# Iselix/kwiiyatta

Measured on AMD Instinct MI355X. Metric: frames/sec end-to-end analyse->align->convert->synth, 48 kHz 5 ms hop, higher is better.
Workload: dtype f64; 1 GPU; config3: 48 kHz source (10 s, T=2001) + target (11 s, T=2201) pairs: CheapTrick+D4C of both, pad with freshly drawn silent spectra, sp2mc, FastDTW(radius 32) align, GMM(64 comp, D=144)+MLPG convert, mc2sp, WORLD synthesis; pairs_per_gpu=32, streams_per_gpu=4, GPU_MAX_HW_QUEUES=4, launch=the whole step is one captured HIP graph, gmm_model_prepared=once per converter (the per-mixture matrices depend on the GMM only), parallelism=pairs in lockstep x32 per GPU, pair-per-GPU x1, no collective

## Files before the change

### kwiiyatta_amd/csrc/kwy_align.hip

```cpp
#include "kwy_internal.hpp"

__device__ __forceinline__ void align_features_body(const double *__restrict__ mc, int64_t T,
                                                    int ncoef, const double *__restrict__ f0,
                                                    double power_threshold, double power_weight,
                                                    double vuv_weight, double *__restrict__ out) {
  __shared__ double red[KWY_WAVES];
  const int tid = threadIdx.x;
  double mx = -INFINITY;
  for (int64_t t = tid; t < T; t += KWY_THREADS) mx = fmax(mx, mc[t * ncoef]);
#pragma unroll
  for (int o = 32; o > 0; o >>= 1) mx = fmax(mx, __shfl_down(mx, o));
  if ((tid & 63) == 0) red[tid >> 6] = mx;
  __syncthreads();
  double m = red[0];
  for (int i = 1; i < KWY_WAVES; ++i) m = fmax(m, red[i]);
  const double thr = m - power_threshold;
  const int64_t t = (int64_t)blockIdx.x * 8 + (tid >> 5);
  if (t >= T) return;
  const int w = ncoef + 1;
  for (int c = tid & 31; c < w; c += 32) {
    double v;
    if (c == 0) v = mc[t * ncoef] >= thr ? power_weight : 0.0;
    else if (c == 1) v = f0[t] > 0 ? vuv_weight : 0.0;
    else v = mc[t * ncoef + (c - 1)];
    out[t * w + c] = v;
  }
}

#define AL_TILE 1024
#define AL_NT 256
__device__ __forceinline__ void align_project_body(const int32_t *__restrict__ path,
                                                   const int64_t *__restrict__ path_len, int trim_len,
                                                   int32_t *__restrict__ idx, int64_t cap,
                                                   int64_t *__restrict__ n_out) {
  __shared__ int32_t sp[2 * AL_TILE];
  __shared__ int32_t so[AL_TILE];
  __shared__ long long st[5];
  __shared__ int s_irregular;
  const int tid = threadIdx.x, lane = tid & 63;
  const int64_t L = *path_len;
  if (L <= 0) { if (tid == 0) *n_out = 0; return; }
  long long len_y = path[2 * (L - 1) + 1] + 1;
  const long long prev_y0 = -1 + (trim_len > 0 ? trim_len : 0);
  if (trim_len > 0) len_y -= trim_len;
  if (tid == 0) s_irregular = 0;
  __syncthreads();
  {
    bool bad = false;
    for (int64_t k = tid; k < L; k += AL_NT) {
      const long long y = path[2 * k + 1], yp = k > 0 ? path[2 * k - 1] : -1;
      if (y < yp || y - yp > 1) bad = true;
    }
    if (bad) s_irregular = 1;
  }
  __syncthreads();
  if (!s_irregular) {
    for (int64_t k = tid; k < L; k += AL_NT) {
      const long long y = path[2 * k + 1], yp = k > 0 ? path[2 * k - 1] : -1;
      if (y > yp && y > prev_y0 && y < len_y) {
        const long long n = y - (prev_y0 + 1);
        if (n < cap) idx[n] = path[2 * k];
      }
    }
    if (tid == 0) { const long long n = len_y - (prev_y0 + 1); *n_out = n > 0 ? n : 0; }
    return;
  }
  if (tid >= 64) return;
  if (lane == 0) { st[0] = -1; st[1] = prev_y0; st[2] = 0; st[3] = 0; st[4] = 0; }
  int64_t k0 = 0;
  while (k0 < L) {
    const int nk = (int)min((int64_t)AL_TILE, L - k0);
    for (int e = lane; e < 2 * nk; e += 64) sp[e] = path[2 * k0 + e];
    __builtin_amdgcn_wave_barrier();
    __threadfence_block();
    __shared__ int s_used, s_made;
    if (lane == 0) {
      long long prev_x = st[0], prev_y = st[1];
      int made = 0, k = 0;
// ... 1 lines not shown
      for (; k < nk && !stop; ++k) {
        long long x = sp[2 * k], y = sp[2 * k + 1];
        if (y <= prev_y) continue;
        if (y - prev_y > 1) {
          if (y > len_y - 1) y = len_y - 1;
          const long long diff_x = x - prev_x, diff_y = y - prev_y;
          long long i = st[4];
          for (; i < diff_y && made < AL_TILE; ++i) {
            const long long den = diff_y - 1, num = diff_x * i;
            const long long q = den != 0 ? (num >= 0 ? num / den : -((-num + den - 1) / den)) : 0;
            so[made++] = (int32_t)(prev_x + q);
          }
          if (i < diff_y) { st[4] = i; break; }
          st[4] = 0;
        } else if (y >= len_y) {
          stop = true;
          break;
        } else {
          if (made >= AL_TILE) break;
          so[made++] = (int32_t)x;
        }
        prev_x = x;
        prev_y = y;
      }
      st[0] = prev_x; st[1] = prev_y;
      s_used = k; s_made = made;
      if (stop) st[3] = 1;
    }
    __builtin_amdgcn_wave_barrier();
    __threadfence_block();
    const int made = s_made, used = s_used;
    const long long n0 = st[2];
    for (int e = lane; e < made; e += 64)
      if (n0 + e < cap) idx[n0 + e] = so[e];
    __builtin_amdgcn_wave_barrier();
    if (lane == 0) st[2] = n0 + made;
    __builtin_amdgcn_wave_barrier();
    __threadfence_block();
    if (st[3]) break;
    if (used == 0 && made == 0) break;
    k0 += used;
  }
  if (lane == 0) *n_out = st[2];
}

#define AL_BATCH 64
template <class JOB>
struct al_jobs { int n; JOB j[AL_BATCH]; };

__global__ __launch_bounds__(KWY_THREADS) void k_align_features(al_jobs<kwy_align_job> b, int ncoef,
                                                               double power_threshold, double power_weight,
                                                               double vuv_weight) {
  const kwy_align_job &q = b.j[blockIdx.y];
  if ((int64_t)blockIdx.x * 8 >= q.T) return;
  align_features_body(q.mc, q.T, ncoef, q.f0, power_threshold, power_weight, vuv_weight, q.out);
}

__global__ __launch_bounds__(AL_NT) void k_align_project(al_jobs<kwy_project_job> b, int trim_len) {
  const kwy_project_job &q = b.j[blockIdx.x];
  align_project_body(q.path, q.path_len, trim_len, q.idx, q.idx_capacity, q.n_out);
}

__global__ void k_gather_rows(al_jobs<kwy_gather_job> b, int width) {
  const kwy_gather_job &q = b.j[blockIdx.y];
  const double *__restrict__ src = q.src;
  const int32_t *__restrict__ idx = q.idx;
  double *__restrict__ dst = q.dst;
  const int64_t src_rows = q.src_rows, n = q.n;
  const int64_t row = blockIdx.x;
  if (row >= n) return;
  int64_t r = idx[row];
  if (r < 0) r = 0;
  if (r >= src_rows) r = src_rows - 1;
  const double *s = src + r * width;
  double *d = dst + row * width;
  for (int c = threadIdx.x; c < width; c += blockDim.x) d[c] = s[c];
}

template <class JOB, class LAUNCH>
static int al_for_batches(const JOB *jobs, int count, LAUNCH launch) {
  for (int j0 = 0; j0 < count; j0 += AL_BATCH) {
    al_jobs<JOB> b;
    b.n = count - j0 < AL_BATCH ? count - j0 : AL_BATCH;
    for (int k = 0; k < AL_BATCH; ++k) b.j[k] = jobs[j0 + (k < b.n ? k : 0)];
    launch(b);
  }
  return KWY_OK;
}

extern "C" int kwy_align_features_batch_dev(kwy_ctx *ctx, const kwy_align_job *jobs, int count, int ncoef,
                                            double power_weight, double power_threshold, double vuv_weight) {
  if (!ctx) return KWY_EINVAL;
  if (!jobs || count < 0 || ncoef < 1) { ctx->err = "align_features: bad argument"; return KWY_EINVAL; }
  for (int j = 0; j < count; ++j)
    if (!jobs[j].mc || !jobs[j].f0 || !jobs[j].out || jobs[j].T <= 0) { ctx->err = "align_features: bad argument"; return KWY_EINVAL; }
  KWY_HIP(hipSetDevice(ctx->device));
  al_for_batches(jobs, count, [&](const al_jobs<kwy_align_job> &b) {
    int64_t T = 0;
    for (int k = 0; k < b.n; ++k) T = b.j[k].T > T ? b.j[k].T : T;
    hipLaunchKernelGGL(k_align_features, dim3((unsigned)((T + 7) / 8), b.n), dim3(KWY_THREADS), 0, ctx->stream, b, ncoef,
                       power_threshold, power_weight, vuv_weight);
  });
  KWY_HIP(hipGetLastError());
  return KWY_OK;
}

extern "C" int kwy_align_features_dev(kwy_ctx *ctx, const double *mc, int64_t T, int ncoef, const double *f0,
                                      double power_weight, double power_threshold, double vuv_weight,
                                      double *out) {
  const kwy_align_job job = {mc, f0, T, out};
  return kwy_align_features_batch_dev(ctx, &job, 1, ncoef, power_weight, power_threshold, vuv_weight);
}

extern "C" int kwy_align_project_batch_dev(kwy_ctx *ctx, const kwy_project_job *jobs, int count, int trim_len) {
  if (!ctx) return KWY_EINVAL;
  if (!jobs || count < 0 || trim_len < 0) { ctx->err = "align_project: bad argument"; return KWY_EINVAL; }
  for (int j = 0; j < count; ++j)
    if (!jobs[j].path || !jobs[j].path_len || !jobs[j].idx || !jobs[j].n_out || jobs[j].idx_capacity <= 0) {
      ctx->err = "align_project: bad argument";
      return KWY_EINVAL;
    }
  KWY_HIP(hipSetDevice(ctx->device));
  al_for_batches(jobs, count, [&](const al_jobs<kwy_project_job> &b) {
    hipLaunchKernelGGL(k_align_project, dim3(b.n), dim3(AL_NT), 0, ctx->stream, b, trim_len);
  });
  KWY_HIP(hipGetLastError());
  return KWY_OK;
}

extern "C" int kwy_align_project_dev(kwy_ctx *ctx, const int32_t *path, const int64_t *path_len, int trim_len,
                                     int32_t *idx, int64_t idx_capacity, int64_t *n_out) {
  const kwy_project_job job = {path, path_len, idx, idx_capacity, n_out};
  return kwy_align_project_batch_dev(ctx, &job, 1, trim_len);
}

extern "C" int kwy_gather_rows_batch_dev(kwy_ctx *ctx, const kwy_gather_job *jobs, int count, int width) {
  if (!ctx) return KWY_EINVAL;
  if (!jobs || count < 0 || width <= 0) { ctx->err = "gather_rows: bad argument"; return KWY_EINVAL; }
  for (int j = 0; j < count; ++j)
    if (!jobs[j].src || !jobs[j].idx || !jobs[j].dst || jobs[j].src_rows <= 0 || jobs[j].n < 0) {
      ctx->err = "gather_rows: bad argument";
      return KWY_EINVAL;
    }
  KWY_HIP(hipSetDevice(ctx->device));
  al_for_batches(jobs, count, [&](const al_jobs<kwy_gather_job> &b) {
    int64_t n = 0;
    for (int k = 0; k < b.n; ++k) n = b.j[k].n > n ? b.j[k].n : n;
    if (n > 0)
      hipLaunchKernelGGL(k_gather_rows, dim3((unsigned)n, b.n), dim3(width >= 256 ? 256 : 64), 0, ctx->stream, b, width);
  });
  KWY_HIP(hipGetLastError());
  return KWY_OK;
}
// ... 7 lines not shown
```

### kwiiyatta_amd/csrc/kwy_dtw.hip

```cpp
#include <math.h>

#include <algorithm>
#include <vector>

#include "kwy_internal.hpp"


__global__ void k_dtw_halve(const double *__restrict__ in, int n_out, int dim, double *__restrict__ out) {
  const int64_t e = (int64_t)blockIdx.x * blockDim.x + threadIdx.x;
  if (e >= (int64_t)n_out * dim) return;
  const int i = (int)(e / dim), k = (int)(e % dim);
  out[e] = (in[(int64_t)(2 * i) * dim + k] + in[(int64_t)(2 * i + 1) * dim + k]) / 2;
}

#define DTW_MAXLV 12

__device__ __forceinline__ int dtw_strip_steps16(const int32_t *lo, const int32_t *hi, int len_x, int k) {
  const int il = min(64 * k + 63, len_x - 1);
  return ((hi[il] - lo[64 * k] + 1 + 63) + 15) & ~15;
}
__device__ __forceinline__ uint64_t dtw_skew_index(uint64_t sbase, int s, int lane) {
  return sbase + ((uint64_t)(s >> 1) * 64 + (uint64_t)lane) * 2 + (uint64_t)(s & 1);
}
template <int NT>
// ... 7 lines not shown
  int32_t *firstj = (int32_t *)(tot + NT), *lastj = firstj + crows;
  if (table) {
    for (int p = threadIdx.x; p < cn; p += NT) {
      const int r = cpath[2 * p], j = cpath[2 * p + 1];
      if (p == 0 || cpath[2 * (p - 1)] != r) firstj[r] = j;
      if (p == cn - 1 || cpath[2 * (p + 1)] != r) lastj[r] = j;
    }
    __syncthreads();
  }
  for (int i = threadIdx.x; i < len_x; i += NT) {
    int l = 0, h = len_y - 1;
    if (table) {
      const int a = i / 2;
      const int fr = a - radius;
      const int jf = fr < crows ? firstj[max(fr, 0)] : lastj[crows - 1];
      const int jl = lastj[min(a + radius, crows - 1)];
      l = max(0, 2 * (jf - radius));
      h = min(len_y - 1, 2 * (jl + radius) + 1);
    } else if (cpath && cn > 0) {
      const int a = i / 2;
      int b0 = 0, b1 = cn;
      while (b0 < b1) { int mid = (b0 + b1) >> 1; if (cpath[2 * mid] >= a - radius) b1 = mid; else b0 = mid + 1; }
      const int first = min(b0, cn - 1);
      b0 = 0; b1 = cn;
      while (b0 < b1) { int mid = (b0 + b1) >> 1; if (cpath[2 * mid] > a + radius) b1 = mid; else b0 = mid + 1; }
      const int last = max(b0 - 1, 0);
      l = max(0, 2 * (cpath[2 * first + 1] - radius));
      h = min(len_y - 1, 2 * (cpath[2 * last + 1] + radius) + 1);
    }
    lo[i] = l;
    hi[i] = h;
  }
  __syncthreads();
  kwy_block_count_scan<NT>([&](int64_t i) -> uint64_t { return (uint64_t)(hi[i] - lo[i] + 1); }, len_x, off, tot);
  const int nstrips = (len_x + 63) / 64;
  kwy_block_count_scan<NT>([&](int64_t k) -> uint64_t { return 64ull * (uint64_t)dtw_strip_steps16(lo, hi, len_x, (int)k); },
                           nstrips, soff, tot);
  __syncthreads();
  if (threadIdx.x == 0 && (off[len_x] > cap_rows || soff[nstrips] > cap_skew)) atomicExch(status, 1);
}

#define DTW_WS_NT 1024
__device__ __forceinline__ void dtw_window_scan_first(int radius, int len_x, int len_y, int32_t *lo, int32_t *hi,
                                                      uint64_t *off, uint64_t *soff, uint64_t cap_rows,
                                                      uint64_t cap_skew, int *status, uint64_t *tot, size_t tot_bytes) {
  if (threadIdx.x < 16) status[threadIdx.x] = 0;
  __syncthreads();
  dtw_window_scan_body<DTW_WS_NT>((const int32_t *)nullptr, 0, radius, len_x, len_y, lo, hi, off, soff, cap_rows,
                                  cap_skew, status, (unsigned char *)tot, tot_bytes);
}

#define DTW_DT 32
#define DTW_DTP (DTW_DT + 1)
#define DTW_DIST_LDS (sizeof(double) * (64 + 80) * DTW_DTP)
__device__ __forceinline__ void dtw_dist_body(const double *x, const double *y, int dim, int len_x, int len_y,
                                              const int32_t *lo, const int32_t *hi, const uint64_t *soff,
                                              double *dist, const int *status, unsigned unit_first,
                                              unsigned unit_stride, unsigned char *lds) {
  double *xs = (double *)lds, *ys = xs + 64 * DTW_DTP;
  if (status[0] != 0) return;
  const int nstrips = (len_x + 63) / 64;
  const uint64_t total = soff[nstrips];
  const int lane = threadIdx.x & 63, sub = threadIdx.x >> 6;
  constexpr int PER = 16 / (KWY_THREADS / 64);
  for (uint64_t cell0 = (uint64_t)unit_first * 1024ull; cell0 < total; cell0 += (uint64_t)unit_stride * 1024ull) {
    int a = 0, b = nstrips - 1;
    while (a < b) { const int mid = (a + b + 1) >> 1; if (soff[mid] <= cell0) a = mid; else b = mid - 1; }
    const int k = a;
    const uint64_t sb = soff[k];
    const int s0 = (int)((cell0 - sb) >> 6);
    const int i = 64 * k + lane;
    const bool valid = i < len_x;
    const int jmin = lo[64 * k], l = valid ? lo[i] : 0, h = valid ? hi[i] : -1;
    const int jbase = jmin + s0 - 63;
    bool in[PER];
    double acc[PER];
    bool any = false;
#pragma unroll
    for (int q = 0; q < PER; ++q) {
      const int j = jmin + s0 + PER * sub + q - lane;
      in[q] = j >= l && j <= h;
      any = any || in[q];
      acc[q] = 0.0;
    }
    if (__syncthreads_or(any)) {
      for (int c0 = 0; c0 < dim; c0 += DTW_DT) {
        const int cw = min(DTW_DT, dim - c0);
        __syncthreads();
        for (int e = threadIdx.x; e < 64 * cw; e += KWY_THREADS) {
          const int r = e / cw, c = e - r * cw, ii = 64 * k + r;
          xs[r * DTW_DTP + c] = ii < len_x ? x[(int64_t)ii * dim + c0 + c] : 0.0;
        }
        for (int e = threadIdx.x; e < 79 * cw; e += KWY_THREADS) {
          const int r = e / cw, c = e - r * cw, jj = jbase + r;
          ys[r * DTW_DTP + c] = (jj >= 0 && jj < len_y) ? y[(int64_t)jj * dim + c0 + c] : 0.0;
        }
        __syncthreads();
#pragma unroll
        for (int q = 0; q < PER; ++q) {
          if (in[q]) {
            const double *xr = xs + lane * DTW_DTP, *yr = ys + (PER * sub + q + 63 - lane) * DTW_DTP;
            double t = acc[q];
            for (int c = 0; c < cw; ++c) { const double df = xr[c] - yr[c]; t += df * df; }
            acc[q] = t;
          }
        }
      }
    }
#pragma unroll
    for (int q = 0; q < PER; ++q)
      dist[dtw_skew_index(sb, s0 + PER * sub + q, lane)] = in[q] ? sqrt(acc[q]) : INFINITY;
    __syncthreads();
  }
}

__device__ __forceinline__ double dtw_wave_shr1(double v, double first) {
  const int lo = __builtin_amdgcn_update_dpp(__double2loint(first), __double2loint(v), 0x138, 0xf, 0xf, false);
  const int hi = __builtin_amdgcn_update_dpp(__double2hiint(first), __double2hiint(v), 0x138, 0xf, 0xf, false);
  return __hiloint2double(hi, lo);
}
__device__ __forceinline__ int dtw_wave_shr1_i32(int v, int first) {
  return __builtin_amdgcn_update_dpp(first, v, 0x138, 0xf, 0xf, false);
}
__device__ __forceinline__ double dtw_wave_rol1(double v) {
  const int lo = __builtin_amdgcn_mov_dpp(__double2loint(v), 0x134, 0xf, 0xf, false);
  const int hi = __builtin_amdgcn_mov_dpp(__double2hiint(v), 0x134, 0xf, 0xf, false);
  return __hiloint2double(hi, lo);
}

__device__ __forceinline__ double dtw_min_raw(double a, double b) {
  return fmin(a, b);
}

__device__ __forceinline__ uint64_t dtw_group_base(const uint64_t *__restrict__ off, int i) {
  return (off[i] >> 6) + (uint64_t)i;
}

struct dtw_level_args {
  int len_x, len_y;
  const int32_t *lo, *hi;
  const uint64_t *off;
  const uint64_t *soff;
  uint64_t cap_rows, cap_skew;
  double *dist;
  double *dval;
  uint64_t *predm;
  double *bnd_global;
  int32_t *path, *rev, *sinfo;
  int64_t *path_len;
  double *out_dist;
  int *status;
  long long *dbg;
  int lds_bytes;
  int next_len_x, next_len_y, radius;
  int32_t *lo_w, *hi_w;
  uint64_t *off_w, *soff_w;
  const double *x, *y;
  int dim;
};

#define DTW_OFFLV 32
struct dtw_pair {
  const double *x, *y;
  int Tx, Ty;
  double *dist;
// ... 7 lines not shown
  uint64_t stride;
  uint64_t cap_rows, cap_skew;
  uint64_t off_x[DTW_OFFLV], off_y[DTW_OFFLV];
  uint64_t off_dist, off_dval, off_soff, off_predm, off_lo, off_hi, off_off, off_bnd, off_pathA, off_pathB, off_rev,
      off_sinfo, off_lenA, off_lenB, off_status;
  int bnd_lds;
  long long *dbg;
  dtw_pair p[KWY_BATCH_MAX];
};
__host__ __device__ static inline int dtw_num_levels(int Tx, int Ty, int radius) {
  int n = 1;
  while (!(Tx < radius + 2 || Ty < radius + 2)) { Tx /= 2; Ty /= 2; ++n; }
  return n;
}
__device__ __forceinline__ bool dtw_make_args(const dtw_batch &b, int pi, int lev, bool with_series, dtw_level_args &a) {
  const dtw_pair &q = b.p[pi];
  const int nlev = dtw_num_levels(q.Tx, q.Ty, b.radius);
  if (lev >= nlev) return false;
  char *base = b.scratch + (uint64_t)pi * b.stride;
  a.len_x = q.Tx >> lev; a.len_y = q.Ty >> lev;
  a.lo = (int32_t *)(base + b.off_lo); a.hi = (int32_t *)(base + b.off_hi);
  a.off = (uint64_t *)(base + b.off_off); a.soff = (uint64_t *)(base + b.off_soff);
  a.cap_rows = b.cap_rows; a.cap_skew = b.cap_skew;
  a.dist = (double *)(base + b.off_dist); a.dval = (double *)(base + b.off_dval);
  a.predm = (uint64_t *)(base + b.off_predm);
  a.bnd_global = b.bnd_lds ? nullptr : (double *)(base + b.off_bnd);
  const bool top = lev == 0;
  a.path = top ? q.path : (int32_t *)(base + ((lev & 1) ? b.off_pathA : b.off_pathB));
  a.path_len = top ? q.path_len : (int64_t *)(base + ((lev & 1) ? b.off_lenA : b.off_lenB));
  a.rev = (int32_t *)(base + b.off_rev); a.sinfo = (int32_t *)(base + b.off_sinfo);
  a.out_dist = q.dist;
  a.status = (int *)(base + b.off_status);
  a.dbg = b.dbg;
  a.lds_bytes = b.lds_bytes;
  a.next_len_x = top ? 0 : q.Tx >> (lev - 1);
  a.next_len_y = top ? 0 : q.Ty >> (lev - 1);
  a.radius = b.radius;
  a.lo_w = (int32_t *)(base + b.off_lo); a.hi_w = (int32_t *)(base + b.off_hi);
  a.off_w = (uint64_t *)(base + b.off_off); a.soff_w = (uint64_t *)(base + b.off_soff);
  a.x = with_series ? (lev == 0 ? q.x : (const double *)(base + b.off_x[lev])) : nullptr;
  a.y = with_series ? (lev == 0 ? q.y : (const double *)(base + b.off_y[lev])) : nullptr;
  a.dim = b.dim;
  return true;
}

#define DTW_WAVES 4
#define DTW_CHUNK 16
#ifndef DTW_RING
#define DTW_RING 5
#endif
#ifndef DTW_BLK
#define DTW_BLK 16
#endif
typedef double dtw_d2 __attribute__((ext_vector_type(2), aligned(16)));

template <bool BND_LDS>
__device__ __forceinline__ void dtw_values_body(const dtw_level_args &a, unsigned char *bt ) {
  const long long t_start = a.dbg ? clock64() : 0;
  __shared__ long long s_prog[DTW_WAVES];
#define DTW_PROG_LOAD(b) __hip_atomic_load(&s_prog[b], __ATOMIC_RELAXED, __HIP_MEMORY_SCOPE_WORKGROUP)
#define DTW_PROG_STORE(b, v) __hip_atomic_store(&s_prog[b], (long long)(v), __ATOMIC_RELAXED, __HIP_MEMORY_SCOPE_WORKGROUP)
#define DTW_RELEASE() do { if (BND_LDS) __builtin_amdgcn_fence(__ATOMIC_RELEASE, "wavefront"); else __builtin_amdgcn_fence(__ATOMIC_RELEASE, "workgroup"); } while (0)
#define DTW_ACQUIRE() do { if (BND_LDS) __builtin_amdgcn_fence(__ATOMIC_ACQUIRE, "wavefront"); else __builtin_amdgcn_fence(__ATOMIC_ACQUIRE, "workgroup"); } while (0)
  const int lane = threadIdx.x & 63, wv = __builtin_amdgcn_readfirstlane(threadIdx.x >> 6);
  if (a.status[0] != 0) return;
  const int len_x = a.len_x, len_y = a.len_y;
  const int32_t *lo = a.lo, *hi = a.hi;
  const uint64_t *off = a.off;
  long long *dbg = a.dbg;
  const double INF = INFINITY;
  const int rowlen = len_y + 2;
  double *const lds_rows = (double *)bt;
  double *const bnd_global = a.bnd_global;
#define BROW(buf, ix) (BND_LDS ? lds_rows[(buf) * rowlen + (ix)] : bnd_global[(size_t)(buf) * rowlen + (ix)])
  if (threadIdx.x < DTW_WAVES) DTW_PROG_STORE(threadIdx.x, -1);
  if (dbg && lane == 0) dbg[16 + wv] = __builtin_amdgcn_s_getreg((31 << 11) | (0 << 6) | 4);
  __syncthreads();
  const int nstrips = (len_x + 63) / 64;
  for (int k = wv; k < nstrips; k += DTW_WAVES) {
    const int i0 = k * 64;
    const int i = i0 + lane;
    const bool valid = i < len_x;
    const int rl = valid ? lo[i] : 0, rh = valid ? hi[i] : -1;
    const int rw = rh - rl;
    const int ilast = min(i0 + 63, len_x - 1);
    const int L = ilast - i0;
    const int jmin = __builtin_amdgcn_readfirstlane(lo[i0]), jmax = __builtin_amdgcn_readfirstlane(hi[ilast]);
    const int plo = k > 0 ? __builtin_amdgcn_readfirstlane(lo[i0 - 1]) : 0;
    const int phi = k > 0 ? __builtin_amdgcn_readfirstlane(hi[i0 - 1]) : -1;
    const int pbuf = (k + DTW_WAVES - 1) % DTW_WAVES, nbuf = k % DTW_WAVES;
    const uint64_t sbv = a.soff[k];
    const uint64_t sb = ((uint64_t)(uint32_t)__builtin_amdgcn_readfirstlane((int)(sbv >> 32)) << 32) |
                        (uint64_t)(uint32_t)__builtin_amdgcn_readfirstlane((int)(uint32_t)sbv);
    const dtw_d2 *dbase = (const dtw_d2 *)(a.dist + sb) + lane;
    dtw_d2 *vbase = (dtw_d2 *)(a.dval + sb) + lane;
    double v1 = INF;
    double up_prev = INF;
    const int nsteps = (jmax - jmin + 1) + 63, nsteps16 = (nsteps + 15) & ~15;
    if (dbg && lane == 0 && k < 48) { dbg[64 + 4 * k] = clock64() - t_start; dbg[64 + 4 * k + 2] = nsteps; dbg[64 + 4 * k + 3] = jmin; }
    const int shift = lane + rl - jmin;
    const int shL = __builtin_amdgcn_readlane(shift, L), rwL = __builtin_amdgcn_readlane(rw, L);
    const int rhL = __builtin_amdgcn_readlane(rh, L);
    int sIn0 = (shL + DTW_BLK - 1) & ~(DTW_BLK - 1);
    const int sIn1 = (shL + rwL - (DTW_BLK - 1)) & ~(DTW_BLK - 1);
    if (sIn1 < sIn0) sIn0 = 0x40000000;
    const unsigned inSpan = sIn1 >= sIn0 ? (unsigned)(sIn1 - sIn0) : 0u;
    if (k == 0 && lane == 0 && jmin == 0) up_prev = 0.0;
// ... 463 lines not shown
  for (int s = sub; s < steps; s += DTW_WAVES) {
    const int j = jmin + s - lane;
    double d = INFINITY;
    if (j >= l && j <= h) {
      const double *yr = ys + j * dp;
      double acc = 0.0;
      for (int c = 0; c < dim; ++c) { const double df = xr[c] - yr[c]; acc += df * df; }
      d = sqrt(acc);
    }
    a.dist[dtw_skew_index(0, s, lane)] = d;
  }
}
__global__ __launch_bounds__(KWY_THREADS) void k_dtw_halve_all(dtw_batch b) {
  extern __shared__ double hb[];
  const dtw_pair &q = b.p[blockIdx.y];
  const int levels = dtw_num_levels(q.Tx, q.Ty, b.radius) - 1;
  if (levels < 1) return;
  const int C = 1 << levels, dim = b.dim;
  const int chunks0 = (q.Tx + C - 1) / C;
  if ((int)blockIdx.x >= chunks0 + (q.Ty + C - 1) / C) return;
  char *base = b.scratch + (uint64_t)blockIdx.y * b.stride;
  const int s = (int)blockIdx.x < chunks0 ? 0 : 1;
  const int c = s == 0 ? blockIdx.x : blockIdx.x - chunks0;
  const int n = s == 0 ? q.Tx : q.Ty;
  const double *src = s == 0 ? q.x : q.y;
  double *A = hb, *B = hb + (size_t)C * dim;
  const int64_t f0 = (int64_t)c * C;
  const int have = (int)min((int64_t)C, (int64_t)n - f0);
  for (int e = threadIdx.x; e < have * dim; e += KWY_THREADS) A[e] = src[f0 * dim + e];
  __syncthreads();
  for (int l = 1; l <= levels; ++l) {
    const int nl = n >> l, per = C >> l;
    const int i0 = c * per;
    const int cnt = min(per, nl - i0);
    double *out = (double *)(base + (s == 0 ? b.off_x[l] : b.off_y[l]));
    for (int e = threadIdx.x; e < cnt * dim; e += KWY_THREADS) {
      const int i = e / dim, k = e - i * dim;
      const double v = (A[(2 * i) * dim + k] + A[(2 * i + 1) * dim + k]) / 2;
      B[e] = v;
      out[(int64_t)(i0 + i) * dim + k] = v;
    }
    __syncthreads();
    double *t = A; A = B; B = t;
  }
}
__global__ __launch_bounds__(DTW_WS_NT) void k_dtw_window_scan(dtw_batch b, int lev) {
  __shared__ uint64_t tot[DTW_WS_NT];
  dtw_level_args a;
  const dtw_pair &q = b.p[blockIdx.x];
  if (lev != dtw_num_levels(q.Tx, q.Ty, b.radius) - 1 || !dtw_make_args(b, blockIdx.x, lev, false, a)) return;
  dtw_window_scan_first(b.radius, a.len_x, a.len_y, a.lo_w, a.hi_w, a.off_w, a.soff_w, a.cap_rows, a.cap_skew, a.status,
                        tot, sizeof(tot));
}
__global__ __launch_bounds__(KWY_THREADS) void k_dtw_dist(dtw_batch b, int lev) {
  __shared__ double tiles[(64 + 80) * DTW_DTP];
  dtw_level_args a;
  if (!dtw_make_args(b, blockIdx.y, lev, true, a)) return;
  dtw_dist_body(a.x, a.y, a.dim, a.len_x, a.len_y, a.lo, a.hi, a.soff, a.dist, a.status, blockIdx.x, gridDim.x,
                (unsigned char *)tiles);
}
template <bool BND_LDS>
__global__ __launch_bounds__(64 * DTW_WAVES) void k_dtw_values(dtw_batch b, int lev) {
  extern __shared__ unsigned char bt[];
  dtw_level_args a;
  if (!dtw_make_args(b, blockIdx.x, lev, false, a)) return;
  dtw_values_body<BND_LDS>(a, bt);
}
__global__ __launch_bounds__(DTW_CODES_THREADS) void k_dtw_codes(dtw_batch b, int lev) {
  extern __shared__ unsigned char bt[];
  dtw_level_args a;
  if (!dtw_make_args(b, blockIdx.y, lev, false, a)) return;
  if ((int)blockIdx.x >= (a.len_x + 63) / 64) return;
  dtw_codes_body<DTW_CODES_THREADS>(a, blockIdx.x, bt);
}
__global__ __launch_bounds__(DTW_TRACE_NT) void k_dtw_trace(dtw_batch b, int lev) {
  extern __shared__ unsigned char bt[];
  dtw_level_args a;
  if (!dtw_make_args(b, blockIdx.x, lev, false, a)) return;
  dtw_trace_body(a, bt);
}
__global__ __launch_bounds__(64 * DTW_WAVES) void k_dtw_small(dtw_batch b, int lev, int with_dist) {
  extern __shared__ unsigned char bt[];
  dtw_level_args a;
  if (!dtw_make_args(b, blockIdx.x, lev, with_dist != 0, a)) return;
  if (a.x) { dtw_dist_small(a, bt); __syncthreads(); }
  dtw_values_body<true>(a, bt);
  __syncthreads();
  const int nstrips = (a.len_x + 63) / 64;
  for (int k = 0; k < nstrips; ++k) dtw_codes_body<64 * DTW_WAVES>(a, k, bt);
  __syncthreads();
  dtw_trace_body(a, bt);
}

static uint64_t dtw_cap(int len_x, int len_y, int radius, bool full) {
  const uint64_t worst = (uint64_t)len_x * (uint64_t)len_y;
  if (full) return worst;
  const uint64_t r = (uint64_t)radius;
  const uint64_t bound = 2 * (2 * r + 1) * ((uint64_t)len_y + 2) + ((uint64_t)len_x + 2) * (4 * r + 2);
  return bound < worst ? bound : worst;
}
static uint64_t dtw_cap_skew(int len_x, int len_y, int radius, bool full) {
  const uint64_t strips = ((uint64_t)len_x + 63) / 64;
  const uint64_t worst = 64 * strips * ((uint64_t)len_y + 80);
  if (full) return worst;
  const uint64_t r = (uint64_t)radius, m = (31 + 2 * r) / 32 + 1;
  const uint64_t bound = 64 * (m * ((uint64_t)len_y + 2) + strips * (4 * r + 2 + 63 + 15 + 16));
  return bound < worst ? bound : worst;
}
// ... 44 lines not shown
  b.dbg = (long long *)ctx->dbg;
  for (int p = 0; p < n; ++p) status_out[p] = (int *)(b.scratch + (size_t)p * b.stride + b.off_status);
  int nlev[KWY_BATCH_MAX], top = 0;
  for (int p = 0; p < n; ++p) { nlev[p] = dtw_num_levels(pairs[p].Tx, pairs[p].Ty, radius); top = std::max(top, nlev[p]); }
  {
    const int levels = top - 1;
    const size_t halve_lds = levels > 0 ? sizeof(double) * (((size_t)3 << levels) / 2) * dim : 0;
    if (levels > 0 && levels <= DTW_MAXLV && halve_lds <= 64 * 1024) {
      unsigned chunks = 1;
      for (int p = 0; p < n; ++p) {
        const int C = 1 << (nlev[p] - 1);
        chunks = std::max(chunks, (unsigned)((pairs[p].Tx + C - 1) / C + (pairs[p].Ty + C - 1) / C));
      }
      hipLaunchKernelGGL(k_dtw_halve_all, dim3(chunks, n), dim3(KWY_THREADS), halve_lds, ctx->stream, b);
    } else {
      for (int p = 0; p < n; ++p) {
        const double *px = pairs[p].x, *py = pairs[p].y;
        char *base = b.scratch + (size_t)p * b.stride;
        for (int l = 1; l < nlev[p]; ++l) {
          const int lx = pairs[p].Tx >> l, ly = pairs[p].Ty >> l;
          double *cx = (double *)(base + b.off_x[l]), *cy = (double *)(base + b.off_y[l]);
          hipLaunchKernelGGL(k_dtw_halve, dim3((unsigned)(((size_t)lx * dim + 255) / 256)), dim3(256), 0, ctx->stream, px,
                             lx, dim, cx);
          hipLaunchKernelGGL(k_dtw_halve, dim3((unsigned)(((size_t)ly * dim + 255) / 256)), dim3(256), 0, ctx->stream, py,
                             ly, dim, cy);
          px = cx; py = cy;
        }
      }
    }
  }
  const size_t bnd_bytes = sizeof(double) * DTW_WAVES * (Ty + 2);
  b.bnd_lds = bnd_bytes <= 150 * 1024 ? 1 : 0;
  const size_t big_lds = 150 * 1024;
  KWY_HIP(hipFuncSetAttribute((const void *)k_dtw_values<true>, hipFuncAttributeMaxDynamicSharedMemorySize, (int)big_lds));
  KWY_HIP(hipFuncSetAttribute((const void *)k_dtw_codes, hipFuncAttributeMaxDynamicSharedMemorySize, (int)big_lds));
  KWY_HIP(hipFuncSetAttribute((const void *)k_dtw_trace, hipFuncAttributeMaxDynamicSharedMemorySize, (int)big_lds));
  KWY_HIP(hipFuncSetAttribute((const void *)k_dtw_small, hipFuncAttributeMaxDynamicSharedMemorySize, (int)big_lds));

  for (int l = top - 1; l >= 0; --l) {
    int len_x = 0, len_y = 0;
    bool first = false, small = b.bnd_lds != 0, small_dist = true;
    for (int p = 0; p < n; ++p) {
      if (l >= nlev[p]) continue;
      const int lx = pairs[p].Tx >> l, ly = pairs[p].Ty >> l;
      len_x = std::max(len_x, lx); len_y = std::max(len_y, ly);
      first = first || l == nlev[p] - 1;
      small = small && (lx + 63) / 64 <= DTW_SMALL_STRIPS;
      small_dist = small_dist && sizeof(double) * (size_t)(lx + ly) * (size_t)(dim | 1) <= 96 * 1024;
    }
    small_dist = small_dist && small;
    if (first)
      hipLaunchKernelGGL(k_dtw_window_scan, dim3(n), dim3(DTW_WS_NT), 0, ctx->stream, b, l);
    const int nstrips = (len_x + 63) / 64;
    const uint64_t lv_units = std::min(b.cap_skew, dtw_cap_skew(len_x, len_y, radius, full)) / 1024 + 1;
    b.lds_bytes = 0;
    if (!small_dist)
      KWY_PROF(ctx, "k_dtw_dist", hipLaunchKernelGGL(k_dtw_dist, dim3((unsigned)lv_units, n), dim3(KWY_THREADS), 0, ctx->stream, b, l));
    if (small) {
      const size_t dist_b = small_dist ? sizeof(double) * (size_t)(len_x + len_y) * (size_t)(dim | 1) : 0;
      const size_t bnd_b = sizeof(double) * DTW_WAVES * ((size_t)len_y + 2);
      const size_t groups = 64 * ((size_t)len_y / 64 + 2);
      const size_t codes_b = (size_t)64 * 4 * (size_t)std::min<int64_t>(len_y, 8 * (int64_t)radius + 128) + 32 * groups;
      const size_t trace_b = 16 * ((size_t)len_x + 2) + 8 * DTW_TRACE_NT + 16 * groups + 256;
      size_t need = std::max(std::max(dist_b, bnd_b), std::max(codes_b, trace_b)) + 4096;
      need = std::min(big_lds, (need + 1023) & ~(size_t)1023);
      b.lds_bytes = (int)need;
      KWY_PROF(ctx, "k_dtw_small", hipLaunchKernelGGL(k_dtw_small, dim3(n), dim3(64 * DTW_WAVES), need, ctx->stream, b, l,
                                                       small_dist ? 1 : 0));
      continue;
    }
    const size_t want = (size_t)64 * 4 * (size_t)std::min<int64_t>(len_y, 8 * (int64_t)radius + 128);
    const size_t codes_lds = std::min(big_lds, std::max<size_t>(want, 16 * 1024));
    if (b.bnd_lds)
      KWY_PROF(ctx, "k_dtw_values", hipLaunchKernelGGL(k_dtw_values<true>, dim3(n), dim3(64 * DTW_WAVES), bnd_bytes, ctx->stream, b, l));
    else
      KWY_PROF(ctx, "k_dtw_values", hipLaunchKernelGGL(k_dtw_values<false>, dim3(n), dim3(64 * DTW_WAVES), 0, ctx->stream, b, l));
    b.lds_bytes = (int)codes_lds;
    KWY_PROF(ctx, "k_dtw_codes", hipLaunchKernelGGL(k_dtw_codes, dim3(nstrips, n), dim3(DTW_CODES_THREADS), codes_lds, ctx->stream, b, l));
    b.lds_bytes = (int)big_lds;
    KWY_PROF(ctx, "k_dtw_trace", hipLaunchKernelGGL(k_dtw_trace, dim3(n), dim3(DTW_TRACE_NT), big_lds, ctx->stream, b, l));
  }
  KWY_HIP(hipGetLastError());
  return KWY_OK;
}

static int dtw_check(kwy_ctx *ctx, const void *x, int64_t Tx, const void *y, int64_t Ty, int dim, int radius,
                     const void *dist, const void *path, const void *path_len) {
  if (!ctx) return KWY_EINVAL;
  if (!x || !y || !dist || !path || !path_len || Tx <= 0 || Ty <= 0 || dim <= 0 || dim > 4096 || radius < 0 ||
      Tx > 0x3fffffff || Ty > 0x3fffffff) {
    ctx->err = "fastdtw: bad argument";
    return KWY_EINVAL;
  }
  if (radius < 1) { ctx->err = "fastdtw: radius must be >= 1"; return KWY_EINVAL; }
  return KWY_OK;
}

extern "C" int kwy_fastdtw_batch_dev(kwy_ctx *ctx, const kwy_dtw_job *jobs, int count, int dim, int radius) {
  if (!ctx) return KWY_EINVAL;
  if (!jobs || count < 0) { ctx->err = "fastdtw_batch: bad argument"; return KWY_EINVAL; }
  if (count == 0) return KWY_OK;
  int64_t Tx = 0, Ty = 0;
  for (int j = 0; j < count; ++j) {
    KWY_TRY(dtw_check(ctx, jobs[j].x, jobs[j].x_length, jobs[j].y, jobs[j].y_length, dim, radius, jobs[j].dist,
                      jobs[j].path, jobs[j].path_len));
    Tx = std::max(Tx, jobs[j].x_length); Ty = std::max(Ty, jobs[j].y_length);
  }
// ... 60 lines not shown
```

### kwiiyatta_amd/csrc/kwy_synth.hip

```cpp
#include <math.h>
#include <stdlib.h>

#include <algorithm>
#include <vector>

#include "kwy_internal.hpp"

#define SYN_SAFE 0.000000000001
#define SYN_DEFAULT_F0 500.0
#define SYN_TILE_PER_THREAD 4
#define SYN_TILE (KWY_THREADS * SYN_TILE_PER_THREAD)
#define SYN_TWO_PI (2.0 * KWY_PI)
#define SYN_SLOTS(y_length, fs) ((int)((y_length) * 640 / (fs)) + 64)

struct syn_params {
  int64_t T, y_length;
  int fs, fft_size;
  double frame_period;
  double lowest_f0;
  double sp_mul;
};

__device__ __forceinline__ double syn_increment(const double *__restrict__ f0, const syn_params &p,
                                                int64_t n, double *vuv_out) {
// ... 996 lines not shown
          const double im2 = sqrt(1.0 - re2 * re2);
          buf[k] = {__builtin_fma(re, re2, im * im2), __builtin_fma(im, re2, -(re * im2))};
        }
      } else {
#pragma unroll
        for (int r = 0; r < RK; ++r) {
          const int k = tid + NT * r;
          if (k <= H) buf[k] = cmulf(mp[r], buf[k]);
        }
      }
      SYN_STAMP(3 + 5 * part);
      syn_irfft_inplace<LOG2N - 1, NT, V>(buf, twl, twP, twb, twN);
      SYN_STAMP(4 + 5 * part);
      if (part == 0) {
        const double *w = (const double *)buf;
        double ps[V];
#pragma unroll
        for (int g = 0; g < V; ++g) {
          ps[g] = 0.0;
          for (int i = tid + NT * g; i < H; i += KWY_THREADS) ps[g] += w[i];
        }
        dc_component = syn_block_sum_v<NT, V>(ps, red);
        SYN_STAMP(5);
      }
    }
    {
      const int tid = kwy_tid_opaque();
      SYN_STAMP(10);
      const double *w = (const double *)buf;
      const double sqrt_noise_size = sqrt((double)noise_size);
      double *slot = DIRECT ? nullptr : resp + (size_t)(pp - first_pulse) * N;
      const int64_t offset = (int64_t)idx - H + 1;
#pragma unroll
      for (int m = 0; m < C; ++m) {
        int i = tid + NT * m;
        double aper = (i < H) ? w[i + H] : w[i - H];
        double pv = 0.0;
        if (has_periodic) pv = (i < H) ? -dc_component * dc_remover[i] : lap[i - H] - dc_component * dc_remover[i];
        const double r = (pv * sqrt_noise_size + aper) / N;
        if constexpr (DIRECT) {
          const int64_t n = offset + i;
          if (n >= 0 && n < p.y_length) y[n] += r;
        } else {
          slot[i] = r;
        }
      }
      SYN_STAMP(11);
    }
  }
#undef SYN_STAMP
}


__global__ __launch_bounds__(KWY_THREADS) void k_syn_ola(syn_batch batch, int N) {
  const int utt = batch.find(blockIdx.x);
  const double *__restrict__ resp = batch.u[utt].resp;
  const int32_t *__restrict__ pidx = batch.u[utt].pidx;
  const int *__restrict__ tile_off = batch.u[utt].tile_off;
  const int *__restrict__ npulse = batch.u[utt].npulse;
  const int cap = batch.u[utt].cap, nt = batch.u[utt].nt, first_pulse = 0, slots = batch.u[utt].slots;
  const int64_t y_length = batch.u[utt].p.y_length;
  double *__restrict__ y = batch.u[utt].y;
  const int H = N / 2;
  const int tile = (int)blockIdx.x - batch.start[utt];
  const int P = min(npulse[0], cap);
  if (first_pulse >= P && first_pulse > 0) return;
  const int reach = (H + SYN_TILE - 1) / SYN_TILE;
  const int ja = max(0, tile - reach), jb = min(nt - 1, tile + reach);
  int p0 = min(tile_off[ja], P), p1 = jb + 1 < nt ? min(tile_off[jb + 1], P) : P;
  p0 = max(p0, first_pulse);
  p1 = min(p1, first_pulse + slots);
  const int64_t n0 = (int64_t)tile * SYN_TILE + threadIdx.x;
  double v[SYN_TILE_PER_THREAD];
#pragma unroll
  for (int m = 0; m < SYN_TILE_PER_THREAD; ++m) {
    const int64_t n = n0 + KWY_THREADS * m;
    v[m] = (first_pulse > 0 && n < y_length) ? y[n] : 0.0;
  }
  for (int pp = p0; pp < p1; ++pp) {
    const int idx = pidx[pp];
    if (pidx[min(P - 1, pp + 1)] - idx <= 0) continue;
    const double *slot = resp + (size_t)(pp - first_pulse) * N;
    const int64_t base = (int64_t)idx - H + 1;
#pragma unroll
    for (int m = 0; m < SYN_TILE_PER_THREAD; ++m) {
      const int64_t q = n0 + KWY_THREADS * m - base;
      if (q >= 0 && q < N) v[m] += slot[q];
    }
  }
#pragma unroll
  for (int m = 0; m < SYN_TILE_PER_THREAD; ++m) {
    const int64_t n = n0 + KWY_THREADS * m;
    if (n < y_length) y[n] = v[m];
  }
}

static int get_dc_remover(kwy_ctx *ctx, int fft_size, const double **out) {
  std::string key = "dcrem:" + std::to_string(fft_size);
  return kwy_cached_table<double>(ctx, key, [&] {
    std::vector<double> h(fft_size);
    double dc_component = 0.0;
    for (int i = 0; i < fft_size / 2; ++i) {
      h[i] = 0.5 - 0.5 * cos(2.0 * KWY_PI * (i + 1.0) / (1.0 + fft_size));
      h[fft_size - i - 1] = h[i];
      dc_component += h[i] * 2.0;
    }
    for (int i = 0; i < fft_size / 2; ++i) {
      h[i] /= dc_component;
      h[fft_size - i - 1] = h[i];
    }
    return h;
  }, out);
}

template <int LOG2N>
static int launch_pulse(kwy_ctx *ctx, syn_batch &batch) {
  constexpr int N = 1 << LOG2N, H = N / 2, K = H + 1;
  const kwy_c *twH, *twN, *twP;
  const uint4 *poly;
  const double *dcrem;
  KWY_TRY(kwy_get_twiddles(ctx, LOG2N - 1, &twH));
  KWY_TRY(kwy_get_twiddle_powers(ctx, LOG2N - 1, &twP));
  KWY_TRY(kwy_get_twiddles(ctx, LOG2N, &twN));
  KWY_TRY(kwy_get_poly(ctx, 12ull * (N / syn_pulse_nt<LOG2N>::value), &poly));
  KWY_TRY(get_dc_remover(ctx, N, &dcrem));
  constexpr int NT = syn_pulse_nt<LOG2N>::value;
  static_assert(K + 1 == syn_pulse_form<LOG2N>::H + 2, "the log-spectrum rows");
  size_t lds = syn_pulse_form<LOG2N>::lds;
  KWY_HIP(hipFuncSetAttribute((const void *)k_syn_pulse<LOG2N, false>,
                              hipFuncAttributeMaxDynamicSharedMemorySize, (int)lds));
  KWY_HIP(hipFuncSetAttribute((const void *)k_syn_pulse<LOG2N, true>,
                              hipFuncAttributeMaxDynamicSharedMemorySize, (int)lds));
  const int share = batch.n > 1 ? std::max(64, 4096 / batch.n) : 2048;
  int g = 0;
  for (int u = 0; u < batch.n; ++u) { batch.start[u] = g; g += std::max(1, std::min(batch.u[u].slots, share)); }
  batch.start[batch.n] = g;
  KWY_PROF(ctx, "k_syn_pulse", hipLaunchKernelGGL((k_syn_pulse<LOG2N, false>), dim3(g), dim3(NT), lds, ctx->stream, batch,
                     kwy_randn(ctx), poly, twH, twP, twN, dcrem, (long long *)ctx->dbg));
  g = 0;
  for (int u = 0; u < batch.n; ++u) { batch.start[u] = g; g += batch.u[u].nt; }
// ... 301 lines not shown
```

Measured before the change: 2.858 million frames/s.

## Retile DTW distance kernel, batch OLA pulse loads, widen align feature blocks

The DTW distance kernel now gives each work unit a variable run of anti-diagonal steps. It keeps the x rows in registers, accumulates pairs of cells with 2-wide vector stores across column chunks, and finds the strip with a block-parallel search. The synth overlap-add stages pulse indices in shared memory and issues loads for several pulses before accumulating, which raises memory-level parallelism. Align feature extraction now has each block handle 64 frames with a flat, coalesced write loop. These changes cut redundant LDS reloads and serial dependent loads, at the cost of more register pressure and extra read-modify-write passes over the distance buffer for each column chunk.

```diff
diff --git a/kwiiyatta_amd/csrc/kwy_align.hip b/kwiiyatta_amd/csrc/kwy_align.hip
--- a/kwiiyatta_amd/csrc/kwy_align.hip
+++ b/kwiiyatta_amd/csrc/kwy_align.hip
@@ -1,5 +1,8 @@
 #include "kwy_internal.hpp"
 
+#ifndef AL_FEAT_FRAMES
+#define AL_FEAT_FRAMES 64
+#endif
 __device__ __forceinline__ void align_features_body(const double *__restrict__ mc, int64_t T,
                                                     int ncoef, const double *__restrict__ f0,
                                                     double power_threshold, double power_weight,
@@ -7,6 +10,7 @@
   __shared__ double red[KWY_WAVES];
   const int tid = threadIdx.x;
   double mx = -INFINITY;
+#pragma unroll 8
   for (int64_t t = tid; t < T; t += KWY_THREADS) mx = fmax(mx, mc[t * ncoef]);
 #pragma unroll
   for (int o = 32; o > 0; o >>= 1) mx = fmax(mx, __shfl_down(mx, o));
@@ -15,15 +19,23 @@
   double m = red[0];
   for (int i = 1; i < KWY_WAVES; ++i) m = fmax(m, red[i]);
   const double thr = m - power_threshold;
-  const int64_t t = (int64_t)blockIdx.x * 8 + (tid >> 5);
-  if (t >= T) return;
   const int w = ncoef + 1;
-  for (int c = tid & 31; c < w; c += 32) {
+  const int64_t t0 = (int64_t)blockIdx.x * AL_FEAT_FRAMES;
+  const int64_t t1 = t0 + AL_FEAT_FRAMES < T ? t0 + AL_FEAT_FRAMES : T;
+  const int n = (int)(t1 - t0) * w;
+  const int dq = KWY_THREADS / w, dr = KWY_THREADS % w;
+  int tl = tid / w, c = tid % w;
+  double *__restrict__ dst = out + t0 * w;
+#pragma unroll 4
+  for (int e = tid; e < n; e += KWY_THREADS) {
+    const int64_t t = t0 + tl;
     double v;
     if (c == 0) v = mc[t * ncoef] >= thr ? power_weight : 0.0;
     else if (c == 1) v = f0[t] > 0 ? vuv_weight : 0.0;
     else v = mc[t * ncoef + (c - 1)];
-    out[t * w + c] = v;
+    dst[e] = v;
+    tl += dq; c += dr;
+    if (c >= w) { c -= w; ++tl; }
   }
 }
 
@@ -131,7 +143,7 @@
                                                                double power_threshold, double power_weight,
                                                                double vuv_weight) {
   const kwy_align_job &q = b.j[blockIdx.y];
-  if ((int64_t)blockIdx.x * 8 >= q.T) return;
+  if ((int64_t)blockIdx.x * AL_FEAT_FRAMES >= q.T) return;
   align_features_body(q.mc, q.T, ncoef, q.f0, power_threshold, power_weight, vuv_weight, q.out);
 }
 
@@ -177,7 +189,8 @@
   al_for_batches(jobs, count, [&](const al_jobs<kwy_align_job> &b) {
     int64_t T = 0;
     for (int k = 0; k < b.n; ++k) T = b.j[k].T > T ? b.j[k].T : T;
-    hipLaunchKernelGGL(k_align_features, dim3((unsigned)((T + 7) / 8), b.n), dim3(KWY_THREADS), 0, ctx->stream, b, ncoef,
+    hipLaunchKernelGGL(k_align_features, dim3((unsigned)((T + AL_FEAT_FRAMES - 1) / AL_FEAT_FRAMES), b.n), dim3(KWY_THREADS), 0,
+                       ctx->stream, b, ncoef,
                        power_threshold, power_weight, vuv_weight);
   });
   KWY_HIP(hipGetLastError());
diff --git a/kwiiyatta_amd/csrc/kwy_dtw.hip b/kwiiyatta_amd/csrc/kwy_dtw.hip
--- a/kwiiyatta_amd/csrc/kwy_dtw.hip
+++ b/kwiiyatta_amd/csrc/kwy_dtw.hip
@@ -83,65 +83,115 @@
 
 #define DTW_DT 32
 #define DTW_DTP (DTW_DT + 1)
-#define DTW_DIST_LDS (sizeof(double) * (64 + 80) * DTW_DTP)
+#ifndef DTW_RUN
+#define DTW_RUN 64
+#endif
+#define DTW_YROWS (DTW_RUN + 63)
+#define DTW_DIST_ROWS (DTW_YROWS + 1)
+#define DTW_DIST_LDS (sizeof(double) * DTW_DIST_ROWS * DTW_DTP)
+typedef double dtw_d2 __attribute__((ext_vector_type(2), aligned(16)));
+__host__ __device__ static inline uint64_t dtw_dist_units(uint64_t cells, uint64_t strips) {
+  return cells / (64ull * DTW_RUN) + strips + 1;
+}
+template <int CW>
+__device__ __forceinline__ void dtw_dist_pair(const double (&xr)[DTW_DT], const double *yr, double &a0, double &a1) {
+#pragma unroll
+  for (int c = 0; c < CW; ++c) {
+    if (c % 8 == 0) __builtin_amdgcn_sched_barrier(0);
+    const double d0 = xr[c] - yr[c], d1 = xr[c] - yr[DTW_DTP + c];
+    a0 += d0 * d0;
+    a1 += d1 * d1;
+  }
+}
 __device__ __forceinline__ void dtw_dist_body(const double *x, const double *y, int dim, int len_x, int len_y,
                                               const int32_t *lo, const int32_t *hi, const uint64_t *soff,
                                               double *dist, const int *status, unsigned unit_first,
                                               unsigned unit_stride, unsigned char *lds) {
-  double *xs = (double *)lds, *ys = xs + 64 * DTW_DTP;
-  if (status[0] != 0) return;
+  static_assert(DTW_RUN % 16 == 0 && DTW_RUN / 2 % KWY_WAVES == 0 && DTW_DIST_ROWS >= 64, "the run's thread map");
+  static_assert(KWY_THREADS % DTW_DT == 0 && DTW_DIST_ROWS % (8 * (KWY_THREADS / DTW_DT)) == 0, "the staging map");
+  double *tile = (double *)lds;
   const int nstrips = (len_x + 63) / 64;
-  const uint64_t total = soff[nstrips];
+  const int overflow = status[0];
+  const uint64_t nunits = soff[nstrips] / (64ull * DTW_RUN) + (uint64_t)nstrips;
+  if (overflow != 0) return;
   const int lane = threadIdx.x & 63, sub = threadIdx.x >> 6;
-  constexpr int PER = 16 / (KWY_THREADS / 64);
-  for (uint64_t cell0 = (uint64_t)unit_first * 1024ull; cell0 < total; cell0 += (uint64_t)unit_stride * 1024ull) {
+  const int scol = threadIdx.x & (DTW_DT - 1), srow = threadIdx.x / DTW_DT;
+  constexpr int SROWS = KWY_THREADS / DTW_DT;
+  constexpr int XP = 64 / SROWS, YP = DTW_DIST_ROWS / SROWS;
+  for (uint64_t u = unit_first; u < nunits; u += unit_stride) {
     int a = 0, b = nstrips - 1;
-    while (a < b) { const int mid = (a + b + 1) >> 1; if (soff[mid] <= cell0) a = mid; else b = mid - 1; }
-    const int k = a;
-    const uint64_t sb = soff[k];
-    const int s0 = (int)((cell0 - sb) >> 6);
+    while (b - a >= KWY_THREADS) {
+      const int mid = (a + b + 1) >> 1;
+      if (soff[mid] / (64ull * DTW_RUN) + (uint64_t)mid <= u) a = mid; else b = mid - 1;
+    }
+    const int cand = a + (int)threadIdx.x;
+    const int k = a - 1 + __syncthreads_count(cand <= b && soff[cand] / (64ull * DTW_RUN) + (uint64_t)cand <= u);
+    const uint64_t sb = soff[k], sb_next = soff[k + 1];
     const int i = 64 * k + lane;
     const bool valid = i < len_x;
     const int jmin = lo[64 * k], l = valid ? lo[i] : 0, h = valid ? hi[i] : -1;
+    const int steps16 = (int)((sb_next - sb) >> 6);
+    const int s0 = (int)(u - (sb / (64ull * DTW_RUN) + (uint64_t)k)) * DTW_RUN;
+    if (s0 >= steps16) continue;
+    const int nst = min(DTW_RUN, steps16 - s0);
     const int jbase = jmin + s0 - 63;
-    bool in[PER];
-    double acc[PER];
-    bool any = false;
-#pragma unroll
-    for (int q = 0; q < PER; ++q) {
-      const int j = jmin + s0 + PER * sub + q - lane;
-      in[q] = j >= l && j <= h;
-      any = any || in[q];
-      acc[q] = 0.0;
-    }
-    if (__syncthreads_or(any)) {
-      for (int c0 = 0; c0 < dim; c0 += DTW_DT) {
-        const int cw = min(DTW_DT, dim - c0);
-        __syncthreads();
-        for (int e = threadIdx.x; e < 64 * cw; e += KWY_THREADS) {
-          const int r = e / cw, c = e - r * cw, ii = 64 * k + r;
-          xs[r * DTW_DTP + c] = ii < len_x ? x[(int64_t)ii * dim + c0 + c] : 0.0;
+    dtw_d2 *band = (dtw_d2 *)(dist + sb) + lane;
+    for (int c0 = 0; c0 < dim; c0 += DTW_DT) {
+      const int cw = min(DTW_DT, dim - c0), cwp = (cw + 3) & ~3;
+      const bool first = c0 == 0, last = c0 + DTW_DT >= dim;
+      double xv[XP];
+#pragma unroll
+      for (int q = 0; q < XP; ++q) {
+        const int ii = 64 * k + srow + SROWS * q;
+        xv[q] = (scol < cw && ii < len_x) ? x[(int64_t)ii * dim + c0 + scol] : 0.0;
+      }
+      __syncthreads();
+      if (scol < cwp) {
+#pragma unroll
+        for (int q = 0; q < XP; ++q) tile[(srow + SROWS * q) * DTW_DTP + scol] = xv[q];
+      }
+      __syncthreads();
+      double xr[DTW_DT];
+#pragma unroll
+      for (int c = 0; c < DTW_DT; ++c) xr[c] = tile[lane * DTW_DTP + c];
+      __syncthreads();
+      if (scol < cwp) {
+#pragma unroll
+        for (int q0 = 0; q0 < YP; q0 += 8) {
+          double yv[8];
+#pragma unroll
+          for (int q = 0; q < 8; ++q) {
+            const int r = srow + SROWS * (q0 + q), jj = jbase + r;
+            yv[q] = (scol < cw && r < nst + 63 && jj >= 0 && jj < len_y) ? y[(int64_t)jj * dim + c0 + scol] : 0.0;
+          }
+#pragma unroll
+          for (int q = 0; q < 8; ++q) tile[(srow + SROWS * (q0 + q)) * DTW_DTP + scol] = yv[q];
         }
-        for (int e = threadIdx.x; e < 79 * cw; e += KWY_THREADS) {
-          const int r = e / cw, c = e - r * cw, jj = jbase + r;
-          ys[r * DTW_DTP + c] = (jj >= 0 && jj < len_y) ? y[(int64_t)jj * dim + c0 + c] : 0.0;
-        }
-        __syncthreads();
-#pragma unroll
-        for (int q = 0; q < PER; ++q) {
-          if (in[q]) {
-            const double *xr = xs + lane * DTW_DTP, *yr = ys + (PER * sub + q + 63 - lane) * DTW_DTP;
-            double t = acc[q];
-            for (int c = 0; c < cw; ++c) { const double df = xr[c] - yr[c]; t += df * df; }
-            acc[q] = t;
+      }
+      __syncthreads();
+      for (int p = sub; 2 * p < nst; p += KWY_WAVES) {
+        const int j0 = jmin + s0 + 2 * p - lane;
+        const bool in0 = j0 >= l && j0 <= h, in1 = j0 + 1 >= l && j0 + 1 <= h;
+        dtw_d2 *cell = band + (size_t)((s0 >> 1) + p) * 64;
+        double a0 = 0.0, a1 = 0.0;
+        if (in0 || in1) {
+          if (!first) { const dtw_d2 v = *cell; a0 = v.x; a1 = v.y; }
+          const double *yr = tile + (2 * p + 63 - lane) * DTW_DTP;
+          switch (cwp) {
+            case 4: dtw_dist_pair<4>(xr, yr, a0, a1); break;
+            case 8: dtw_dist_pair<8>(xr, yr, a0, a1); break;
+            case 12: dtw_dist_pair<12>(xr, yr, a0, a1); break;
+            case 16: dtw_dist_pair<16>(xr, yr, a0, a1); break;
+            case 20: dtw_dist_pair<20>(xr, yr, a0, a1); break;
+            case 24: dtw_dist_pair<24>(xr, yr, a0, a1); break;
+            case 28: dtw_dist_pair<28>(xr, yr, a0, a1); break;
+            default: dtw_dist_pair<32>(xr, yr, a0, a1); break;
           }
         }
-      }
-    }
-#pragma unroll
-    for (int q = 0; q < PER; ++q)
-      dist[dtw_skew_index(sb, s0 + PER * sub + q, lane)] = in[q] ? sqrt(acc[q]) : INFINITY;
-    __syncthreads();
+        if (last) { a0 = in0 ? sqrt(a0) : INFINITY; a1 = in1 ? sqrt(a1) : INFINITY; }
+        *cell = dtw_d2{a0, a1};
+      }
+    }
   }
 }
 
@@ -255,7 +305,6 @@
 #ifndef DTW_BLK
 #define DTW_BLK 16
 #endif
-typedef double dtw_d2 __attribute__((ext_vector_type(2), aligned(16)));
 
 template <bool BND_LDS>
 __device__ __forceinline__ void dtw_values_body(const dtw_level_args &a, unsigned char *bt ) {
@@ -825,8 +874,8 @@
   dtw_window_scan_first(b.radius, a.len_x, a.len_y, a.lo_w, a.hi_w, a.off_w, a.soff_w, a.cap_rows, a.cap_skew, a.status,
                         tot, sizeof(tot));
 }
-__global__ __launch_bounds__(KWY_THREADS) void k_dtw_dist(dtw_batch b, int lev) {
-  __shared__ double tiles[(64 + 80) * DTW_DTP];
+__global__ __launch_bounds__(KWY_THREADS, 3) void k_dtw_dist(dtw_batch b, int lev) {
+  __shared__ double tiles[DTW_DIST_ROWS * DTW_DTP];
   dtw_level_args a;
   if (!dtw_make_args(b, blockIdx.y, lev, true, a)) return;
   dtw_dist_body(a.x, a.y, a.dim, a.len_x, a.len_y, a.lo, a.hi, a.soff, a.dist, a.status, blockIdx.x, gridDim.x,
@@ -977,7 +1026,8 @@
     if (first)
       hipLaunchKernelGGL(k_dtw_window_scan, dim3(n), dim3(DTW_WS_NT), 0, ctx->stream, b, l);
     const int nstrips = (len_x + 63) / 64;
-    const uint64_t lv_units = std::min(b.cap_skew, dtw_cap_skew(len_x, len_y, radius, full)) / 1024 + 1;
+    const uint64_t lv_units = std::min<uint64_t>(
+        dtw_dist_units(std::min(b.cap_skew, dtw_cap_skew(len_x, len_y, radius, full)), (uint64_t)nstrips), 0x7fffffffull);
     b.lds_bytes = 0;
     if (!small_dist)
       KWY_PROF(ctx, "k_dtw_dist", hipLaunchKernelGGL(k_dtw_dist, dim3((unsigned)lv_units, n), dim3(KWY_THREADS), 0, ctx->stream, b, l));
diff --git a/kwiiyatta_amd/csrc/kwy_synth.hip b/kwiiyatta_amd/csrc/kwy_synth.hip
--- a/kwiiyatta_amd/csrc/kwy_synth.hip
+++ b/kwiiyatta_amd/csrc/kwy_synth.hip
@@ -1072,6 +1072,9 @@
 }
 
 
+#ifndef SYN_OLA_GROUP
+#define SYN_OLA_GROUP 4
+#endif
 __global__ __launch_bounds__(KWY_THREADS) void k_syn_ola(syn_batch batch, int N) {
   const int utt = batch.find(blockIdx.x);
   const double *__restrict__ resp = batch.u[utt].resp;
@@ -1097,15 +1100,36 @@
     const int64_t n = n0 + KWY_THREADS * m;
     v[m] = (first_pulse > 0 && n < y_length) ? y[n] : 0.0;
   }
-  for (int pp = p0; pp < p1; ++pp) {
-    const int idx = pidx[pp];
-    if (pidx[min(P - 1, pp + 1)] - idx <= 0) continue;
-    const double *slot = resp + (size_t)(pp - first_pulse) * N;
-    const int64_t base = (int64_t)idx - H + 1;
-#pragma unroll
-    for (int m = 0; m < SYN_TILE_PER_THREAD; ++m) {
-      const int64_t q = n0 + KWY_THREADS * m - base;
-      if (q >= 0 && q < N) v[m] += slot[q];
+  __shared__ int32_t s_idx[KWY_THREADS + 1];
+  for (int c0 = p0; c0 < p1; c0 += KWY_THREADS) {
+    const int cn = min(KWY_THREADS, p1 - c0);
+    __syncthreads();
+    if ((int)threadIdx.x < cn) s_idx[threadIdx.x] = pidx[min(P - 1, c0 + (int)threadIdx.x)];
+    if (threadIdx.x == 0) s_idx[cn] = pidx[min(P - 1, c0 + cn)];
+    __syncthreads();
+    for (int g0 = 0; g0 < cn; g0 += SYN_OLA_GROUP) {
+      double r[SYN_OLA_GROUP][SYN_TILE_PER_THREAD];
+      bool on[SYN_OLA_GROUP][SYN_TILE_PER_THREAD];
+#pragma unroll
+      for (int g = 0; g < SYN_OLA_GROUP; ++g) {
+        const int e = min(g0 + g, cn - 1);
+        const int idx = s_idx[e];
+        const bool live = g0 + g < cn && s_idx[e + 1] - idx > 0;
+        const double *slot = resp + (size_t)(c0 + e - first_pulse) * N;
+        const int64_t base = (int64_t)idx - H + 1;
+#pragma unroll
+        for (int m = 0; m < SYN_TILE_PER_THREAD; ++m) {
+          const int64_t q = n0 + KWY_THREADS * m - base;
+          on[g][m] = live && q >= 0 && q < N;
+          r[g][m] = on[g][m] ? slot[q] : 0.0;
+        }
+      }
+#pragma unroll
+      for (int g = 0; g < SYN_OLA_GROUP; ++g) {
+#pragma unroll
+        for (int m = 0; m < SYN_TILE_PER_THREAD; ++m)
+          if (on[g][m]) v[m] += r[g][m];
+      }
     }
   }
 #pragma unroll
```

Result: faster. 2.935 million frames/s (median of 6 runs) (+2.7%).
